# mjiUST/SurfaceNet

Hardware: AMD Instinct MI355X
Metric: voxel-cubes/sec (CVC warp + 3D CNN fwd) at s=32, N_viewpair=2 (higher is better)
Workload: dtype f16x3 (each operand = hi+lo fp16 pair, 3 MFMAs per product, f32 accumulate: fp32-class results; the two correction terms of a product run on one MX-scaled MFMA in the two merge layers (fp6 e2m3 codes) and in the three dilated layers conv4_x (fp8 e4m3 codes); L_inf vs fp64 oracle 3e-5 .. 1.7e-4, asse; 1 GPU; synthetic 2-view 1600x1200, s=32, batch=64 cubes/GPU, N_viewpair=2 (BASELINE.json configs[1]); cubes_per_gpu=64, parallelism=cube-sharded x1

## Files before the change

surfacenet_amd/csrc/conv3d_mfma.h:

```cpp
#pragma once
#include <hip/hip_runtime.h>
#include "mx_format.h"
#include <stdint.h>
#include <type_traits>

constexpr int kRowGap3x3 = 4, kRowGap2D = 4, kRowGapDil2 = 2;
#ifndef SN_TIMING
#define SN_TIMING 0
#endif
#define PW_SB __builtin_amdgcn_sched_barrier(0)

namespace sn {

typedef _Float16 half8 __attribute__((ext_vector_type(8)));
typedef _Float16 half4 __attribute__((ext_vector_type(4)));
typedef float f32x4 __attribute__((ext_vector_type(4)));

constexpr int kMaxSlab = 128;

struct ConvArgs {
    const _Float16 *in;
    _Float16 *out;
    float *out_f32;
    const _Float16 *wpack;
    const float *scale;
    const float *shift;
    const float *w3;
    const void *zero_page;
    const _Float16 *side_w;
    const float *side_scale, *side_shift;
    _Float16 *side_out, *pool_out;
    long long side_lo_off, pool_lo_off;
    int side_cs, side_coff, pool_cs, side_act;
    unsigned *status;
    unsigned status_bit;
    unsigned mx_sat_bits;
    float scale3, shift3;
    long long wsplit_stride;
    long long in_lo_off, out_lo_off;
    long long out_code_off;
    int in_cs, out_cs, out_coff, out_cp;
    int D, DX, tiles_x, tiles_y, tiles_z, total_tiles;
    int act;
    int mx_in_e8, mx_out_e8, mx_side_e8;
    int nslab;
    int c8_last;
    int bridge;
};

enum { EPI_STORE = 0, EPI_FINAL = 1, EPI_POOL2D = 2, EPI_SIDEPOOL = 3 };

template <int V> struct IntC { static constexpr int value = V; };
__device__ __forceinline__ float sn_sigmoid(float x) { return 1.0f / (1.0f + __expf(-x)); }
typedef float f32x2_t __attribute__((ext_vector_type(2)));
__device__ __forceinline__ void sn_track_acc(f32x2_t &c, const f32x4 &a)
// ... 93 lines not shown
__device__ __forceinline__ void pw_mfma_f16(f32x4 &c, const half8 &a, const half8 &b)
{
    asm volatile("v_mfma_f32_16x16x32_f16 %0, %1, %2, %0" : "+a"(c) : "v"(a), "v"(b));
}
template <int OPSEL>
__device__ __forceinline__ void pw_mfma_mx6(f32x4 &c, const mx_v6i &a, const mx_v6i &b, int sa, int sb)
{
    static_assert(OPSEL >= 0 && OPSEL < 4, "scale byte");
#define SN_MX6_ASM(SEL) "v_mfma_scale_f32_16x16x128_f8f6f4 %0, %1, %2, %0, %3, %4 " SEL " cbsz:" SN_STR(SN_MX_FMT) " blgp:" SN_STR(SN_MX_FMT)
    if constexpr (OPSEL == 0) asm volatile(SN_MX6_ASM("op_sel_hi:[0,0,0]") : "+a"(c) : "v"(a), "v"(b), "v"(sa), "v"(sb));
    else if constexpr (OPSEL == 1) asm volatile(SN_MX6_ASM("op_sel:[1,0,0] op_sel_hi:[0,0,0]") : "+a"(c) : "v"(a), "v"(b), "v"(sa), "v"(sb));
    else if constexpr (OPSEL == 2) asm volatile(SN_MX6_ASM("op_sel_hi:[1,0,0]") : "+a"(c) : "v"(a), "v"(b), "v"(sa), "v"(sb));
    else asm volatile(SN_MX6_ASM("op_sel:[1,0,0] op_sel_hi:[1,0,0]") : "+a"(c) : "v"(a), "v"(b), "v"(sa), "v"(sb));
#undef SN_MX6_ASM
}
__device__ __forceinline__ void pw_mfma_mx8(f32x4 &c, const v8i &a, const v8i &b, int sa, int sb)
{
    asm volatile("v_mfma_scale_f32_16x16x128_f8f6f4 %0, %1, %2, %0, %3, %4 op_sel_hi:[0,0,0]" : "+a"(c) : "v"(a), "v"(b), "v"(sa), "v"(sb));
}
constexpr unsigned HB_ALWAYS = 1u << 31, HB_XLO = 1u << 30, HB_XHI = 1u << 29, HB_YLO = 1u << 28, HB_YHI = 1u << 27, HB_ZLO = 1u << 26,
                   HB_ZHI = 1u << 25, HB_OFFMASK = (1u << 25) - 1;

template <int KS, int DIL, int MF, int NF, int EPI, int SPLIT, int CS8, int PCH_, int NW_, int PADV_, int K2D = 0>
struct ConvCfg {
    static constexpr int R = (KS / 2) * DIL;
    static constexpr int RX = K2D ? 0 : R;
    static constexpr int XS = MF / 4;
    static constexpr int NW = NW_;
    static constexpr int NT = NW * 64;
    static constexpr bool F4 = (K2D == 2);
    static constexpr int TX = F4 ? NW * MF : NW * XS, TY = F4 ? 4 : 8, TZ = F4 ? 4 : 8;
    static constexpr int HX = TX + 2 * RX, HY = TY + 2 * R, HZ = TZ + 2 * R;
    static constexpr int HVOX = HX * HY * HZ;
    static constexpr int CS8MAX = CS8;
    static constexpr int SLOTS = CS8 + PADV_;
    static constexpr int VS = SLOTS * 16;
    static constexpr int PCH = PCH_;
    static constexpr int NPL = SPLIT ? 2 : 1;
    static constexpr int NPLM = SPLIT == 1 ? 2 : 1;
    static constexpr int FRAG = 1024 * NPL;
    static constexpr int MFRAG = 1024 * NPLM;
    static_assert(SPLIT < 2 || PCH_ == 2, "f16m8: a weight piece is 2 K-chunks + one MX step");
    static constexpr int MXF = SPLIT == 3 ? 0 : SN_MX_FMT;
    static constexpr int WBUF = PCH * NF * FRAG;
    static constexpr int NTAP = (K2D ? 1 : KS) * KS * KS;
    static constexpr int KOFF_N = NTAP * CS8MAX + 24;
    static constexpr bool PWM = (SPLIT == 3 || (SPLIT == 2 && SN_MX_FMT != 0)) && K2D == 0 && NW_ == 4 && KS == 3 && MF == 8 && PCH_ == 2;
    static constexpr int PW_TABS = 16;
    static constexpr int pw_tab(int kb, int slab, bool last) { return kb * PW_TABS + (last ? 8 : 0) + (slab & 7); }
    static constexpr int pw_xoff(int m) { return (((m >> 2) * HY + (m & 3)) * HZ) * VS; }
    static constexpr int XGAP = DIL == 2 ? kRowGapDil2 : kRowGap3x3;
    static constexpr int xoff_of(int m) { return XGAP == 4 ? pw_xoff(m) : (((m >> 2) * HY + (m & 1) + 4 * ((m >> 1) & 1)) * HZ) * VS; }
    static constexpr bool PTAB = SPLIT < 2 && NW_ == 8 && KS == 3 && PCH_ >= 2 && (K2D == 0 || SPLIT != 0) && !PWM;
    static constexpr int KTAB_N = PWM ? PW_TABS * KOFF_N : (PTAB ? 8 * KOFF_N : KOFF_N);
    static constexpr int NSEG0 = (HVOX * VS + 1023) / 1024;
    static constexpr int NSEG = PWM ? (NSEG0 + NW_ - 1) / NW_ * NW_ : NSEG0;
    static constexpr int XPLANE = NSEG * 1024;
    static constexpr int XBUF = XPLANE * NPL;
#ifndef SN_PW_WB3
#define SN_PW_WB3 0
#endif
    static constexpr bool CST_LDS = (EPI == EPI_STORE) && NF >= 7;
    static constexpr int EPI_CONST = CST_LDS ? NF * 16 * 4 * 2 : 0;
    static constexpr int NWB = (SN_PW_WB3 && PWM && 2 * XBUF + 3 * WBUF + 2 * KTAB_N * 4 + EPI_CONST <= 160 * 1024) ? 3 : 2;
    static constexpr int wb_next(int b) { return NWB == 3 ? (b == 2 ? 0 : b + 1) : (b ^ 1); }
    static constexpr int LDS_BYTES = 2 * XBUF + NWB * WBUF + 2 * KTAB_N * 4 + EPI_CONST;
    static_assert(LDS_BYTES <= 160 * 1024, "LDS budget exceeded");
    static constexpr int WG_PER_CU = (LDS_BYTES <= 80 * 1024 && NW == 4 && MF * NF <= 32) ? 2 : 1;
    static constexpr int MIN_WAVES_PER_SIMD = (NW == 8 || WG_PER_CU == 2) ? 2 : 1;
};

template <int KS, int SPLIT, int NW, int PCH, int NF, int K2D, int MF = 4>
constexpr bool sn_conv_has_bridge()
{
    return (SPLIT == 1 && NW == 8 && KS == 3 && PCH >= 2) ||
           (SPLIT == 2 && K2D == 0 && NW == 8 && KS == 3 && SN_MX_FMT != 0) ||
           ((SPLIT == 3 || (SPLIT == 2 && SN_MX_FMT != 0)) && K2D == 0 && NW == 4 && MF == 8 && KS == 3 && PCH == 2);
}

template <int KS, int DIL, int MF, int NF, int EPI, int SPLIT, int CS8, int PCH_, int NW_, int PADV_, int K2D = 0, int OSPLIT_ = -1>
__global__ void __launch_bounds__(NW_ * 64, (ConvCfg<KS, DIL, MF, NF, EPI, SPLIT, CS8, PCH_, NW_, PADV_, K2D>::MIN_WAVES_PER_SIMD))
conv3d_f16_mfma(ConvArgs a)
{
    constexpr int OSPLIT = OSPLIT_ < 0 ? SPLIT : OSPLIT_;
    using C = ConvCfg<KS, DIL, MF, NF, EPI, SPLIT, CS8, PCH_, NW_, PADV_, K2D>;
    constexpr int NPL = C::NPL;
    __shared__ __attribute__((aligned(16))) char lds[C::LDS_BYTES];
    char *const xbuf = lds;
    char *const wbuf = lds + 2 * C::XBUF;
    int *const kbuf = reinterpret_cast<int *>(lds + 2 * C::XBUF + C::NWB * C::WBUF);
    float *const cst = reinterpret_cast<float *>(lds + 2 * C::XBUF + C::NWB * C::WBUF + 2 * C::KTAB_N * 4);

    const int tid = threadIdx.x, lane = tid & 63, wave = __builtin_amdgcn_readfirstlane(tid >> 6);
    const int v = lane & 15, kq = lane >> 4;
    int mx_sb = a.mx_in_e8;
    if constexpr (SPLIT == 3 || (SPLIT == 2 && SN_MX_FMT != 0)) asm volatile("" : "+v"(mx_sb));
    const int D = a.D, DX = a.DX;
    const size_t VOL = (size_t)DX * D * D;
    const int tstride = gridDim.x;
    auto slab_c8_of = [&](int sl) -> int { return sl + 1 == a.nslab ? a.c8_last : C::CS8MAX; };
    int tile = ((gridDim.x & 7) == 0) ? (int)((blockIdx.x & 7) * (gridDim.x >> 3) + (blockIdx.x >> 3)) : (int)blockIdx.x;
    if (tile >= a.total_tiles) return;

    const char *const wsrc0 = reinterpret_cast<const char *>(a.wpack + (size_t)blockIdx.y * a.wsplit_stride);

    auto tile_origin = [&](int t, int &b, int &x0, int &y0, int &z0) {
        const int tz = t % a.tiles_z; t /= a.tiles_z;
        const int ty = t % a.tiles_y; t /= a.tiles_y;
        const int tx = t % a.tiles_x;
        b = t / a.tiles_x;
        x0 = tx * C::TX; y0 = ty * C::TY; z0 = tz * C::TZ;
// ... 54 lines not shown
            }
            hword[k] = o;
        });
    }
    auto tile_halo_consts = [&](int x0, int y0, int z0, unsigned &keep, int &toff) {
        unsigned inv = K2D ? 0u : HB_ALWAYS;
        if constexpr (K2D == 0) {
            if (x0 == 0) inv |= HB_XLO;
            if (x0 == (a.tiles_x - 1) * C::TX) inv |= HB_XHI;
        }
        if (y0 == 0) inv |= FB_YLO;
        if (y0 == (a.tiles_y - 1) * C::TY) inv |= FB_YHI;
        if (z0 == 0) inv |= FB_ZLO;
        if (z0 == (a.tiles_z - 1) * C::TZ) inv |= FB_ZHI;
        keep = FB_OFFMASK | inv;
        toff = K2D ? ((y0 - C::R) * D + (z0 - C::R)) * 16 : (((x0 - C::RX) * D + (y0 - C::R)) * D + (z0 - C::R)) * 16;
    };
    auto stage_halo_buf = [&](int b, unsigned keep, int toff, int c0, int c8n, int xb, int kb = 0, int ke = 1 << 20) -> int {
        if constexpr (UNI) {
            b = __builtin_amdgcn_readfirstlane(b); keep = __builtin_amdgcn_readfirstlane(keep);
            toff = __builtin_amdgcn_readfirstlane(toff); c0 = __builtin_amdgcn_readfirstlane(c0);
        }
        asm volatile("" : "+s"(b), "+s"(keep), "+s"(toff), "+s"(c0));
        const char *base0;
        int nrec;
        if constexpr (K2D == 0) {
            base0 = reinterpret_cast<const char *>(a.in) + 2 * ((size_t)b * VOL * a.in_cs + (size_t)c0 * VOL * 8);
            nrec = c8n * (int)VOL * 16;
        } else {
            base0 = reinterpret_cast<const char *>(a.in) + 2 * ((size_t)c0 * VOL * 8 + (size_t)b * D * D * 8);
            nrec = (c8n * (int)VOL - b * D * D) * 16;
        }
        if constexpr (UNI) {
            const unsigned long long bq = (unsigned long long)(size_t)base0;
            base0 = (const char *)(size_t)(((unsigned long long)(unsigned)__builtin_amdgcn_readfirstlane((int)(bq >> 32)) << 32) |
                                           (unsigned)__builtin_amdgcn_readfirstlane((int)bq));
            nrec = __builtin_amdgcn_readfirstlane(nrec);
        }
        int issued = 0;
        static_for<0, HT>([&](auto kc) {
            constexpr int k = decltype(kc)::value;
            const int li = k * C::NW + wave;
            if ((k + 1 < HT || C::NSEG * NPL == HT * C::NW || li < C::NSEG * NPL) && k >= kb && k < ke) {
                const char *base = (NPL > 1 && li >= C::NSEG) ? base0 + 2 * a.in_lo_off : base0;
                const __amdgpu_buffer_rsrc_t rs = __builtin_amdgcn_make_buffer_rsrc((void *)base, (short)0, nrec, 0x00020000);
                dma16_buf(rs, (hword[k] & keep) + (unsigned)toff, xbuf + xb * C::XBUF + li * 1024);
                ++issued;
            }
        });
        return issued;
    };
    auto wg_barrier = [&]() { asm volatile("s_barrier" ::: "memory"); };
    constexpr bool BRIDGE_OK = (PPX && SPLIT == 1) || PPM || PWM;
    constexpr int UM = SPLIT >= 2 ? 8 : 4;
    constexpr int BSTEP = (UM - (C::NTAP * C::CS8MAX) % UM) % UM;
    const bool bridge = BRIDGE_OK && a.bridge != 0;
    auto slab_units = [&](int c8n, int slab, int &o, int &b) {
        const int GU = C::NTAP * c8n;
        o = 0; b = 0;
        if (bridge) {
            o = (slab * ((UM - (GU & (UM - 1))) & (UM - 1))) & (UM - 1);
            b = (slab + 1 == a.nslab) ? 0 : ((UM - ((GU - o) & (UM - 1))) & (UM - 1));
        }
        return GU - o + b;
    };
    auto chunks_of = [&](int c8n, int slab) { int o, b; return (slab_units(c8n, slab, o, b) + 3) >> 2; };
    auto wchunks_of = [&](int c8n, int slab) { int o, b; return SPLIT >= 2 ? (((slab_units(c8n, slab, o, b) + 7) >> 3) << 1) : chunks_of(c8n, slab); };
    const int wchunk0 = wchunks_of(slab_c8_of(0), 0);
    auto write_koff_part = [&](int c8n, int kb, int slab, int t0, int nt) {
        int uo, ub;
        const int own = slab_units(c8n, slab, uo, ub) - ub, nchunk = (own + ub + 3) >> 2;
        int *k = kbuf + (PWM ? C::pw_tab(kb, slab, slab + 1 == a.nslab) : (C::PTAB ? kb * 8 + ((slab + 1 == a.nslab) ? 4 : 0) + (slab & 3) : kb)) * C::KOFF_N;
        for (int g = t0; g < (nchunk + 4) * 4; g += nt) {
            int o = 0;
            if (g < own + ub) {
                const int u = g < own ? g + uo : g - own;
                const int far = g < own ? 0 : (1 - 2 * kb) * C::XBUF;
                const int tap = C::CS8MAX == 1 ? u : u / c8n, c8 = C::CS8MAX == 1 ? 0 : u - tap * c8n;
                const int dz = tap % KS, dy = (tap / KS) % KS, dx = tap / (KS * KS);
                o = ((dx * DIL * C::HY + dy * DIL) * C::HZ + dz * DIL) * C::VS + c8 * 16 + far;
            }
            k[g] = o;
        }
    };
    auto write_koff = [&](int c8n, int kb, int slab) { write_koff_part(c8n, kb, slab, tid, C::NT); };
    auto stage_w = [&](size_t off, int nch, int wbi) {
        const int cnt = nch * NF * NPL;
        const char *src = wsrc0 + off;
        char *dst = wbuf + wbi * C::WBUF;
        for (int i = wave; i < cnt; i += C::NW) dma16(src + (size_t)i * 1024 + lane * 16, dst + i * 1024);
    };

    constexpr bool PMAP = (EPI == EPI_SIDEPOOL);
    static_assert(!PMAP || ((MF == 4 || MF == 8) && NW_ == 8 && K2D == 0), "EPI_SIDEPOOL: 8 waves x 4 (8) fragments over an 8x8x8 (16x8x8) tile");
    auto frag_xyz = [&](int m, int &hx, int &hy, int &hz) {
        if constexpr (C::F4) { hx = wave * MF + m; hy = v >> 2; hz = v & 3; }
        else if constexpr (PMAP) { hx = (MF / 2) * (wave & 3) + (m >> 1); hy = 2 * (wave >> 2) + (m & 1) + 4 * (v >> 3); hz = v & 7; }
        else if constexpr (K2D == 0 && KS == 3 && C::XGAP == 4) { hx = wave * C::XS + (m >> 2); hy = (m & 3) + 4 * (v >> 3); hz = v & 7; }
        else if constexpr (K2D == 0 && KS == 3 && C::XGAP == 2) { hx = wave * C::XS + (m >> 2); hy = (m & 1) + 4 * ((m >> 1) & 1) + 2 * (v >> 3); hz = v & 7; }
        else if constexpr (K2D == 1 && kRowGap2D == 4 && C::VS == 32) { hx = wave * C::XS + (m >> 2); hy = (m & 3) + 4 * (v >> 3); hz = v & 7; }
        else { hx = wave * C::XS + (m >> 2); hy = 2 * (m & 3) + (v >> 3); hz = v & 7; }
    };
    int xbase[MF];
#pragma unroll
    for (int m = 0; m < MF; ++m) {
        int hx, hy, hz;
        frag_xyz(m, hx, hy, hz);
        xbase[m] = ((hx * C::HY + hy) * C::HZ + hz) * C::VS;
    }
    const unsigned xbuf_a = lds_addr(xbuf), wbuf_a = lds_addr(wbuf) + lane * 16, kbuf_a = lds_addr(kbuf) + kq * 4;

    if constexpr (C::CST_LDS)
        for (int i = tid; i < NF * 16; i += C::NT) {
            cst[i] = a.scale[blockIdx.y * NF * 16 + i];
            cst[NF * 16 + i] = a.shift[blockIdx.y * NF * 16 + i];
        }
    constexpr int NQ = (NF + 1) / 2;
    half8 sw[EPI == EPI_SIDEPOOL ? NQ : 1][2];
    if constexpr (EPI == EPI_SIDEPOOL) {
#pragma unroll
        for (int q = 0; q < NQ; ++q) {
            sw[q][0] = *reinterpret_cast<const half8 *>(a.side_w + ((size_t)(q * 2 + 0) * 64 + lane) * 8);
            sw[q][1] = *reinterpret_cast<const half8 *>(a.side_w + ((size_t)(q * 2 + 1) * 64 + lane) * 8);
        }
    }
    {
        const int c8n = slab_c8_of(0);
        if constexpr (BUFH) {
            int b, x0, y0, z0, toff;
            unsigned keep;
            tile_origin(tile, b, x0, y0, z0);
            tile_halo_consts(x0, y0, z0, keep, toff);
            stage_halo_buf(K2D ? x0 : b, keep, toff, 0, c8n, 0);
        } else stage_halo(tile, 0, c8n, 0, 0, HT);
        if constexpr (C::PTAB) {
            for (int kb = 0; kb < 2; ++kb)
// ... 1018 lines not shown
```

surfacenet_amd/csrc/sn_api.hip:

```cpp
#include "sn_internal.h"

enum Kind { K_CONV3, K_CONV1, K_DIL3, K_DIL1, K_UP };
struct LayerSpec { const char *name; Kind kind; int cin, cout, act; const char *input; };
static const LayerSpec kSpecs[] = {
    {"conv1_1", K_CONV3, 6, 32, 0, nullptr},       {"conv1_2", K_CONV3, 32, 32, 0, "conv1_1"},    {"conv1_3", K_CONV3, 32, 32, 0, "conv1_2"},
    {"side_op1", K_CONV1, 32, 16, 1, "conv1_3"},
    {"conv2_1", K_CONV3, 32, 80, 0, "conv1_3"},    {"conv2_2", K_CONV3, 80, 80, 0, "conv2_1"},    {"conv2_3", K_CONV3, 80, 80, 0, "conv2_2"},
    {"side_op2", K_CONV1, 80, 16, 1, "conv2_3"},   {"side_op2_deconv", K_UP, 3, 2, 0, nullptr},
    {"conv3_1", K_CONV3, 80, 160, 0, "conv2_3"},   {"conv3_2", K_CONV3, 160, 160, 0, "conv3_1"},  {"conv3_3", K_CONV3, 160, 160, 0, "conv3_2"},
    {"side_op3", K_CONV1, 160, 16, 1, "conv3_3"},  {"side_op3_deconv", K_UP, 5, 4, 0, nullptr},
    {"conv4_1", K_DIL3, 160, 300, 0, "conv3_3"},   {"conv4_2", K_DIL3, 300, 300, 0, "conv4_1"},   {"conv4_3", K_DIL3, 300, 300, 0, "conv4_2"},
    {"side_op4", K_DIL1, 300, 16, 1, "conv4_3"},   {"side_op4_deconv", K_UP, 5, 4, 0, nullptr},
    {"merge_conv_a", K_CONV3, 64, 100, 0, nullptr}, {"merge_conv_b", K_CONV3, 100, 100, 0, "merge_conv_a"}, {"merge_conv3", K_CONV1, 100, 1, 1, "merge_conv_b"},
};
static constexpr int kNumSpecs = sizeof(kSpecs) / sizeof(kSpecs[0]);
static constexpr int kNetParams = 98, kAllParams = 105, kDFeature = 258, kHidden = 100;


static unsigned char fp8_e4m3(float v)
{
    if (v != v) return 0x7f;
    const unsigned char sgn = std::signbit(v) ? 0x80 : 0;
    float a = std::fabs(v);
    if (a >= 448.f) return sgn | 0x7e;
    if (a < std::ldexp(1.0f, -10)) return sgn;
    int e;
    std::frexp(a, &e);
    int E = e - 1;
    if (E < -6) E = -6;
    const float q = std::nearbyint(std::ldexp(a, 3 - E));
    int mant = (int)q, be = E + 7;
    if (E == -6 && mant < 8) be = 0;
    else { if (mant == 16) { mant = 8; be += 1; } mant -= 8; }
    if (be > 15 || (be == 15 && mant > 6)) return sgn | 0x7e;
    return sgn | (unsigned char)(be << 3) | (unsigned char)mant;
}

static unsigned char mx6_encode(float v, int fmt)
{
    const int mb = fmt == 2 ? 3 : 2, bias = fmt == 2 ? 1 : 3, emax = fmt == 2 ? 3 : 7;
    const float vmax = std::ldexp((float)((2 << mb) - 1), emax - bias - mb);
    if (v != v) return 0;
    const unsigned char sgn = std::signbit(v) ? 0x20 : 0;
    float a = std::min(std::fabs(v), vmax);
    int e;
    std::frexp(a, &e);
    int E = (a > 0.f) ? e - 1 : 1 - bias;
    if (E < 1 - bias) E = 1 - bias;
    int mant = (int)std::nearbyint(std::ldexp(a, mb - E));
    int be = E + bias;
    if (mant < (1 << mb)) be = 0;
    else { if (mant == (2 << mb)) { mant = 1 << mb; be += 1; } mant -= 1 << mb; }
    if (be > emax) { be = emax; mant = (1 << mb) - 1; }
    return sgn | (unsigned char)(be << mb) | (unsigned char)mant;
}
static float mx6_max(int fmt) { return fmt == 2 ? 7.5f : 28.f; }

static int pack_conv_host(PackedConv &L, const float *W_in, const float *beta, const float *gamma, const float *mean,
                          const float *inv_std, int nf, int nsplit, int cs8max, int split, const int *in_exp, const int *out_exp,
                          std::vector<_Float16> &h, std::vector<float> &sc, std::vector<float> &sh)
{
    L.nf = nf; L.nsplit = nsplit; L.cs8max = cs8max; L.split = split;
    L.cin_p = round_up(L.cin, 8);
    const int ntap = (L.k2d ? 1 : L.ks) * L.ks * L.ks;
    const int c8_total = L.cin_p / 8;
    const int npl = split == 1 ? 2 : 1;
    L.slab_c8.clear();
    for (int left = c8_total; left > 0; left -= cs8max) L.slab_c8.push_back((unsigned char)std::min(left, cs8max));
    if ((int)L.slab_c8.size() > kMaxSlab) return fail(SN_ERR_ARG, "%s: too many channel slabs", L.name.c_str());
    std::vector<float> Wn((size_t)L.cout * L.cin * ntap);
    std::vector<int> row_exp(L.cout, 0);
    for (int o = 0; o < L.cout; ++o) {
        float mx = 0.f;
        for (int ci = 0; ci < L.cin; ++ci)
            for (int t = 0; t < ntap; ++t) {
                const size_t i = ((size_t)o * L.cin + ci) * ntap + t;
                const float w = in_exp ? std::ldexp(W_in[i], -in_exp[ci]) : W_in[i];
                if (!std::isfinite(w)) return fail(SN_ERR_ARG, "%s: non-finite weight (output channel %d, input channel %d)", L.name.c_str(), o, ci);
                Wn[i] = w;
                mx = std::max(mx, std::fabs(w));
            }
        if (mx > 0.f) row_exp[o] = -std::ilogb(mx);
        if (row_exp[o] != 0)
            for (size_t i = (size_t)o * L.cin * ntap; i < (size_t)(o + 1) * L.cin * ntap; ++i) Wn[i] = std::ldexp(Wn[i], row_exp[o]);
    }
    if (ntap == 1) L.w_norm = Wn;
    const float *W = Wn.data();
    auto wat = [&](int o, int c8abs, int j, int tap) -> float {
        const int ci = c8abs * 8 + j;
        return (o < L.cout && ci < L.cin) ? W[((size_t)o * L.cin + ci) * ntap + tap] : 0.f;
    };
    h.clear();
    {
        const int um = split >= 2 ? 8 : 4;
        bool ok = L.bridge && (split == 1 || (split >= 2 && !L.k2d)) && L.ks == 3 && L.slab_c8.size() >= 2 && (ntap * cs8max) % um != 0;
        for (unsigned char c8n : L.slab_c8) ok = ok && c8n == cs8max;
        L.bridge = ok ? 1 : 0;
    }
    const int nslab = (int)L.slab_c8.size();
    auto slab_units = [&](int si, int c8n, int &o, int &b) {
        const int GU = ntap * c8n, um = split >= 2 ? 8 : 4;
        o = 0; b = 0;
        if (L.bridge) { o = (si * ((um - GU % um) % um)) % um; b = (si + 1 == nslab) ? 0 : (um - (GU - o) % um) % um; }
        return GU - o + b;
    };
    if (split < 2) {
        long long chunks = 0;
        for (int si = 0; si < nslab; ++si) { int o, b; chunks += (slab_units(si, L.slab_c8[si], o, b) + 3) / 4; }
        L.wsplit_stride = chunks * nf * 512 * npl;
        h.assign((size_t)L.wsplit_stride * nsplit, (_Float16)0.f);
        for (int ns = 0; ns < nsplit; ++ns) {
            _Float16 *dst = h.data() + (size_t)ns * L.wsplit_stride;
            int c8_0 = 0;
            for (int si = 0; si < nslab; ++si) {
                const int c8n = L.slab_c8[si];
                int uo, ub;
                const int own = slab_units(si, c8n, uo, ub) - ub, nchunk = (own + ub + 3) / 4;
                for (int ch = 0; ch < nchunk; ++ch)
                    for (int f = 0; f < nf; ++f)
                        for (int lane = 0; lane < 64; ++lane) {
                            const int o = (ns * nf + f) * 16 + (lane & 15);
                            const int g = 4 * ch + (lane >> 4);
                            _Float16 *d8 = dst + (((size_t)ch * nf + f) * npl * 64 + lane) * 8;
                            if (g >= own + ub) continue;
                            const int u = g < own ? g + uo : g - own;
                            const int cb = g < own ? c8_0 : c8_0 + c8n;
                            for (int j = 0; j < 8; ++j) {
                                const float w = wat(o, cb + u % c8n, j, u / c8n);
                                const _Float16 hi = (_Float16)w;
                                d8[j] = hi;
                                if (split == 1) d8[512 + j] = (_Float16)(w - (float)hi);
                            }
                        }
                dst += (size_t)nchunk * nf * 512 * npl;
                c8_0 += c8n;
            }
        }
    } else {
        long long pieces = 0;
        for (int si = 0; si < nslab; ++si) { int o, b; pieces += (slab_units(si, L.slab_c8[si], o, b) + 7) / 8; }
        const size_t piece_halfs = (size_t)nf * 2048;
        L.wsplit_stride = pieces * piece_halfs;
        h.assign((size_t)L.wsplit_stride * nsplit, (_Float16)0.f);
        for (int ns = 0; ns < nsplit; ++ns) {
            _Float16 *dst = h.data() + (size_t)ns * L.wsplit_stride;
            int c8_0 = 0;
            for (int si = 0; si < nslab; ++si) {
                const int c8n = L.slab_c8[si];
                int uo, ub;
                const int own = slab_units(si, c8n, uo, ub) - ub, G = own + ub, npiece = (G + 7) / 8;
                auto wslot = [&](int o, int g, int j) -> float {
                    const int u = g < own ? g + uo : g - own, cb = g < own ? c8_0 : c8_0 + c8n;
                    return wat(o, cb + u % c8n, j, u / c8n);
                };
                for (int p = 0; p < npiece; ++p, dst += piece_halfs) {
                    for (int cc = 0; cc < 2; ++cc)
                        for (int f = 0; f < nf; ++f)
                            for (int lane = 0; lane < 64; ++lane) {
                                const int o = (ns * nf + f) * 16 + (lane & 15);
                                const int g = 8 * p + 4 * cc + (lane >> 4);
                                if (g >= G) continue;
                                _Float16 *d8 = dst + (((size_t)cc * nf + f) * 64 + lane) * 8;
                                for (int j = 0; j < 8; ++j) d8[j] = (_Float16)wslot(o, g, j);
                            }
                    unsigned char *mx = reinterpret_cast<unsigned char *>(dst + (size_t)2 * nf * 512);
                    for (int f = 0; f < nf; ++f)
                        for (int lane = 0; lane < 64; ++lane) {
                            const int o = (ns * nf + f) * 16 + (lane & 15), q = lane >> 4;
                            unsigned char *frag = mx + (size_t)f * 2048;
                            if (split == 2) {
                                float val[32];
                                float amax = 0.f;
                                for (int i = 0; i < 2; ++i) {
                                    const int g = 8 * p + 2 * q + i;
                                    for (int pos = 0; pos < 16; ++pos) {
                                        const int j = (pos & 3) + 4 * (pos >> 3);
                                        const bool lo_part = !(pos & 4);
                                        float t = 0.f;
                                        if (g < G) {
                                            const float w = wslot(o, g, j);
                                            const float hi = (float)(_Float16)w;
                                            t = lo_part ? (w - hi) * kMxLoMul : hi;
                                        }
                                        val[i * 16 + pos] = t;
                                        amax = std::max(amax, std::fabs(t));
                                    }
                                }
                                int E = 0;
                                if (amax > 0.f) {
                                    E = std::ilogb(amax / mx6_max(SN_MX_FMT));
                                    if (std::ldexp(amax, -E) > mx6_max(SN_MX_FMT)) ++E;
                                }
                                E = std::max(-100, std::min(100, E));
                                unsigned w6[6] = {0u, 0u, 0u, 0u, 0u, 0u};
                                for (int el = 0; el < 32; ++el) {
                                    const unsigned code = mx6_encode(std::ldexp(val[el], -E), SN_MX_FMT);
                                    const int bit = 6 * el;
                                    w6[bit >> 5] |= code << (bit & 31);
                                    if ((bit & 31) > 26) w6[(bit >> 5) + 1] |= code >> (32 - (bit & 31));
                                }
                                unsigned *d0 = reinterpret_cast<unsigned *>(frag + lane * 16), *d1 = reinterpret_cast<unsigned *>(frag + 1024 + lane * 16);
                                d0[0] = w6[0]; d0[1] = w6[1]; d0[2] = w6[2]; d0[3] = w6[3];
                                d1[0] = w6[4]; d1[1] = w6[5];
                                (mx + 1024 + lane * 16 + 8)[f] = (unsigned char)std::max(0, std::min(254, 127 + E - kMxLoExp));
                                continue;
// ... 1163 lines not shown
int sn_mark(sn_ctx *c, int slot)
{
    if (!c || slot < 0 || slot >= 8) return fail(SN_ERR_ARG, "sn_mark: slot must be 0..7");
    HIPCHK(hipSetDevice(c->device));
    if (!c->marks[slot]) HIPCHK(hipEventCreateWithFlags(&c->marks[slot], hipEventDisableTiming));
    HIPCHK(hipEventRecord(c->marks[slot], c->stream));
    return SN_OK;
}

int sn_memcpy_d2h_after(sn_ctx *c, int slot, void *dst, const void *src, size_t bytes)
{
    if (!c || !dst || !src) return fail(SN_ERR_ARG, "null argument");
    if (slot < 0 || slot >= 8 || !c->marks[slot]) return fail(SN_ERR_STATE, "sn_memcpy_d2h_after: slot %d was never marked", slot);
    HIPCHK(hipSetDevice(c->device));
    if (!c->copy_stream) HIPCHK(hipStreamCreateWithFlags(&c->copy_stream, hipStreamNonBlocking));
    HIPCHK(hipStreamWaitEvent(c->copy_stream, c->marks[slot], 0));
    HIPCHK(hipMemcpyAsync(dst, src, bytes, hipMemcpyDeviceToHost, c->copy_stream));
    HIPCHK(hipStreamSynchronize(c->copy_stream));
    return SN_OK;
}

#ifdef SN_DEBUG_HOOKS
SN_API int sn_debug_tensor(sn_ctx *c, const char *name, void *host, size_t bytes)
{
    if (!c || !name || !host) return fail(SN_ERR_ARG, "null argument");
    const _Float16 *p = !strcmp(name, "cat") ? c->cat : (!strcmp(name, "ma") ? c->ma : nullptr);
    if (!p) return fail(SN_ERR_ARG, "unknown tensor %s", name);
    HIPCHK(hipSetDevice(c->device));
    HIPCHK(hipStreamSynchronize(c->stream));
    HIPCHK(hipMemcpy(host, p, bytes, hipMemcpyDeviceToHost));
    return SN_OK;
}

SN_API int sn_debug_pack_host(int cin, int cout, int ks, int dil, int k2d, int nf, int nsplit, int cs8max, int split, const float *W, const float *beta,
                              const float *gamma, const float *mean, const float *inv_std, unsigned long long *out)
{
    if (!W || !beta || !gamma || !mean || !inv_std || !out) return fail(SN_ERR_ARG, "null argument");
    PackedConv L;
    L.name = "debug"; L.cin = cin; L.cout = cout; L.ks = ks; L.dil = dil; L.k2d = k2d;
    L.bridge = 1;
    std::vector<_Float16> h;
    std::vector<float> sc, sh;
    const int rc = pack_conv_host(L, W, beta, gamma, mean, inv_std, nf, nsplit, cs8max, split, nullptr, nullptr, h, sc, sh);
    if (rc != SN_OK) return rc;
    unsigned long long sum = 0;
    const unsigned char *b = reinterpret_cast<const unsigned char *>(h.data());
    for (size_t i = 0; i < h.size() * sizeof(_Float16); ++i) sum = sum * 1099511628211ull + b[i];
    out[0] = h.size(); out[1] = sc.size(); out[2] = sh.size(); out[3] = sum;
    return SN_OK;
}

SN_API int sn_debug_plan(int net, int mode, int conv4_fp8, char *rows, int cap)
{
    if (!rows || cap < 1 || net < 0 || net > 1) return fail(SN_ERR_ARG, "sn_debug_plan: bad argument");
    sn_ctx st;
    int rc = sn_set_precision(&st, mode), n = 0;
    if (rc == SN_OK && conv4_fp8 >= 0) rc = sn_set_conv4_fp8(&st, conv4_fp8);
    if (rc != SN_OK) return rc;
    for (const ConvEntry &e : net == 0 ? build_plan(st.split, st.tail_m8, st.c4_m8).conv : simil_plan(st.split)) {
        n += snprintf(rows + n, (size_t)(cap - n), "%s %d %d %d %d %d %d %d %d %d %d %d %d\n", e.name, e.cin, e.cout, e.k.ks, e.k.dil, e.k.k2d,
                      e.k.nf, e.k.nsplit(e.cout), e.k.cs8max, e.k.split, e.k.osplit, e.k.epi, e.bridge);
        if (n >= cap) return fail(SN_ERR_ARG, "sn_debug_plan: the rows do not fit %d bytes", cap);
    }
    return SN_OK;
}

SN_API int sn_debug_mx6_encode(float v, int fmt) { return (fmt == 2 || fmt == 3) ? (int)mx6_encode(v, fmt) : -1; }

SN_API int sn_debug_timing(sn_ctx *c, unsigned long long *out, int n_layers, char *names, int names_cap)
{
    if (!c || !out || !c->d_num) return fail(SN_ERR_ARG, "null argument");
    HIPCHK(hipStreamSynchronize(c->stream));
    n_layers = std::min(n_layers, 32);
    HIPCHK(hipMemcpy(out, c->d_num + 2, sizeof(unsigned long long) * 4 * n_layers, hipMemcpyDeviceToHost));
    HIPCHK(hipMemset(c->d_num + 2, 0, sizeof(unsigned) * 32 * 8));
    std::string all;
    for (auto &nm : c->num_names) all += nm + ",";
    if (names && names_cap > 0) { strncpy(names, all.c_str(), names_cap - 1); names[names_cap - 1] = 0; }
    return SN_OK;
}
SN_API int sn_debug_trace(sn_ctx *c, long long *out)
{
    if (!c || !out || !c->d_num) return fail(SN_ERR_ARG, "null argument");
    HIPCHK(hipStreamSynchronize(c->stream));
    HIPCHK(hipMemcpy(out, c->d_num + 2 + 32 * 8, sizeof(long long) * 2048 * 8 * 2, hipMemcpyDeviceToHost));
    return SN_OK;
}

#endif

int sn_profile_enable(sn_ctx *c, int on)
{
    if (!c) return fail(SN_ERR_ARG, "null context");
    int rc = prof_drain(c);
    c->prof_on = on != 0;
    return rc;
}
int sn_profile_reset(sn_ctx *c)
{
    if (!c) return fail(SN_ERR_ARG, "null context");
    int rc = prof_drain(c);
    for (auto &st : c->prof_stats) { st.ms = 0; st.launches = 0; st.flops = 0; st.bytes = 0; }
    return rc;
}
int sn_profile_count(sn_ctx *c)
{
    if (!c) return fail(SN_ERR_ARG, "null context");
    if (prof_drain(c) != SN_OK) return SN_ERR_HIP;
    return (int)c->prof_stats.size();
}
int sn_profile_get(sn_ctx *c, int idx, char *name, int name_cap, double *ms_total, int64_t *launches, double *flops, double *bytes)
// ... 16 lines not shown
```

surfacenet_amd/csrc/sn_internal.h:

```cpp
#pragma once
#include <hip/hip_runtime.h>
#include <dlfcn.h>

#include <algorithm>
#include <chrono>
#include <cmath>
#include <condition_variable>
#include <memory>
#include <mutex>
#include <thread>
#include <type_traits>
#include <cstdarg>
#include <cstdio>
#include <cstring>
#include <map>
#include <string>
#include <vector>

#include "../../include/surfacenet_hip.h"
#include "conv3d_mfma.h"
#include "cvc_warp.h"
#include "elementwise.h"

using namespace sn;

inline thread_local std::string g_err;

static int fail(int code, const char *fmt, ...)
{
    char buf[1024];
    va_list ap;
    va_start(ap, fmt);
    vsnprintf(buf, sizeof buf, fmt, ap);
    va_end(ap);
    g_err = buf;
    return code;
}

#define HIPCHK(expr)                                                                                       \
    do {                                                                                                   \
        hipError_t e_ = (expr);                                                                            \
        if (e_ != hipSuccess) return fail(SN_ERR_HIP, "%s failed: %s (%s:%d)", #expr, hipGetErrorString(e_), __FILE__, __LINE__); \
    } while (0)


static inline int round_up(int x, int m) { return (x + m - 1) / m * m; }


struct PackedConv {
    std::string name;
    int cin = 0, cout = 0, ks = 1, dil = 1, act = 0;
    int cin_p = 0;
    int nf = 0, nsplit = 1;
    int cs8max = 4, split = 0, k2d = 0;
    int bridge = 0;
    std::vector<unsigned char> slab_c8;
    long long wsplit_stride = 0;
    _Float16 *wpack = nullptr;
    float *scale = nullptr, *shift = nullptr;
    double macs_per_voxel = 0;
    std::vector<float> w_norm;
    _Float16 *side_frag = nullptr;
};

struct sn_ctx;
enum MxExp : unsigned char { MX_ACT, MX_CAT, MX_X0, MX_C4 };

struct Act { _Float16 *p; long long lo; long long code = 0; MxExp e8 = MX_ACT; };

struct SideFuse { const PackedConv *side; Act side_out; int side_cs, side_coff; Act pool_out; int pool_cs; };

struct ConvGeom {
    int ks, dil, k2d, nf, cs8max, split, osplit, epi;
    bool has_bridge;
    int (*launch)(sn_ctx *c, const PackedConv &L, Act in, int in_cs, Act out, int out_cs, int out_coff, int out_cp, float *out_f32, int B, int D, int DX, const SideFuse *sf);
    int nsplit(int cout) const { return ((cout + 15) / 16 + nf - 1) / nf; }
};

struct ConvEntry {
    const char *name; int cin, cout, act;
    ConvGeom k;
    int bridge;
    unsigned char in = 0, out = 0, pool_out = 0;
    const char *pool_tag = nullptr;
    bool up3 = false;
};
struct TensorSpec { _Float16 *sn_ctx::*buf; int level, ch; MxExp e8; int code; };
struct NetPlan {
    int split = -1, tail_m8 = 0, c4_m8 = 0;
    std::vector<ConvEntry> conv;
    std::vector<TensorSpec> tens;
    int (*pool)(sn_ctx *, const char *, Act, Act, int, int, int) = nullptr;
    int (*up3)(sn_ctx *, Act, Act, Act, Act, int, int, int) = nullptr;
};

struct ProfRec { int tag; hipEvent_t e0, e1; double flops, bytes; };
struct ProfStat { std::string name; double ms = 0; int64_t launches = 0; double flops = 0, bytes = 0; };

static inline const char *sn_ab_switch(const char *name)
{
#ifdef SN_DEBUG_HOOKS
    return getenv(name);
#else
    (void)name;
    return nullptr;
#endif
}

constexpr int CC_ERR_INPUT_FLAG = 2;

struct sn_ctx {
    int device = 0, s = 32, max_samples = 0;
    hipStream_t stream = nullptr;
    hipStream_t copy_stream = nullptr;
    hipEvent_t marks[8] = {};
    int V_img = 0, V_cam = 0;
    uint8_t *img_base = nullptr; long long *img_off = nullptr; int *img_h = nullptr, *img_w = nullptr;
    double *cams = nullptr;
    bool have_weights = false, have_relw = false;
    int split = 1;
    int mode = 1;
    int mx_c4_e8 = kMxC4E8;
    int c4_m8 = 1;
    _Float16 *a3c = nullptr;
    int mx_act_e8 = kMxActE8, mx_cat_e8 = kMxCatE8;
    int tail_m8 = 2;
    bool ws_ready = false; int ws_split = -1;
    int last_run_samples = 0;
    NetPlan plan;
// ... 143 lines not shown
                return fail(SN_ERR_ARG, "%s: volume extent %d is not supported by this kernel's halo addressing (extent mod 8 must be 0 or >= %d)", L.name.c_str(), D, C::R);
            const long long plane = (long long)DX * D * D * 16, slack = 4LL * C::HVOX * 16;
            if (K2D == 0 && C::CS8MAX * plane + slack >= (1LL << 25))
                return fail(SN_ERR_ARG, "%s: a %d-group channel slab of a %dx%dx%d volume exceeds the 32 MiB this kernel's halo addressing covers", L.name.c_str(), C::CS8MAX, DX, D, D);
            if (K2D != 0 && SPLIT != 0 && C::CS8MAX * plane + slack >= 0x0FFFFFF0LL - (1 << 16))
                return fail(SN_ERR_ARG, "%s: %d images of %dx%d exceed the 256 MiB this kernel's halo addressing covers per channel slab", L.name.c_str(), DX, D, D);
        }
        a.act = L.act;
        if (EPI == EPI_STORE && KS != 1 && L.act != 0)
            return fail(SN_ERR_STATE, "%s: a sigmoid activation is only built for the 1x1x1 store kernels", L.name.c_str());
        a.mx_in_e8 = mx_e8(c, in.e8); a.mx_out_e8 = mx_e8(c, out.e8); a.mx_side_e8 = mx_e8(c, sf ? sf->side_out.e8 : MX_ACT);
        if (EPI == EPI_SIDEPOOL) {
            if (!sf || !sf->side || !sf->side->side_frag || sf->side->cin != L.cout || sf->side->cout != 16 || L.nsplit != 1 || L.act != 0 || (D & 1))
                return fail(SN_ERR_STATE, "%s: fused side-conv / pool epilogue misconfigured", L.name.c_str());
            a.side_w = sf->side->side_frag; a.side_scale = sf->side->scale; a.side_shift = sf->side->shift; a.side_act = sf->side->act;
            a.side_out = sf->side_out.p; a.side_lo_off = sf->side_out.lo; a.side_cs = sf->side_cs; a.side_coff = sf->side_coff;
            a.pool_out = sf->pool_out.p; a.pool_lo_off = sf->pool_out.lo; a.pool_cs = sf->pool_cs;
        }
        if (c->d_num) {
            auto it = std::find(c->num_names.begin(), c->num_names.end(), L.name);
            size_t bit = it - c->num_names.begin();
            if (it == c->num_names.end() && c->num_names.size() < 31) c->num_names.push_back(L.name);
            a.status = c->d_num;
            constexpr int OS = OSPLIT < 0 ? SPLIT : OSPLIT;
            if (EPI == EPI_STORE && OS >= 2 && L.act == 0) {
                const _Float16 lim = (_Float16)std::min(60000.f, std::ldexp(OS >= 3 ? 255.875f : (SN_MX_FMT == 2 ? 7.5f : 28.f), a.mx_out_e8 - 127));
                unsigned short bits; memcpy(&bits, &lim, 2);
                a.mx_sat_bits = bits;
            }
            a.status_bit = bit < 31 ? (1u << bit) : (1u << 31);
        }
        a.nslab = (int)L.slab_c8.size();
        if (a.nslab < 1) return fail(SN_ERR_STATE, "%s: no channel slabs", L.name.c_str());
        a.bridge = L.bridge;
        if (L.bridge && !geom.has_bridge)
            return fail(SN_ERR_STATE, "%s: packed with bridge chunks, launched on a kernel without them", L.name.c_str());
        if (C::PWM) {
            for (unsigned char c8n : L.slab_c8)
                if (C::NTAP * c8n < 9) return fail(SN_ERR_STATE, "%s: a channel slab of fewer than two weight pieces", L.name.c_str());
        }
        for (int i = 0; i + 1 < a.nslab; ++i)
            if (L.slab_c8[i] != C::CS8MAX) return fail(SN_ERR_STATE, "%s: channel slab %d holds %d groups, the kernel expects %d in all but the last", L.name.c_str(), i, (int)L.slab_c8[i], C::CS8MAX);
        a.c8_last = L.slab_c8.back();
        const double vox = (double)B * DX * D * D;
        const double bytes = vox * 2.0 * (SPLIT ? 2 : 1) * (L.cin + (EPI == EPI_FINAL ? 2 : (EPI == EPI_SIDEPOOL ? 16 + L.cout / 8.0 : L.cout)));
        ProfScope ps(c, L.name, 2.0 * L.macs_per_voxel * vox, bytes);
        const int resident = std::max(1, c->num_cus * C::WG_PER_CU / L.nsplit);
        dim3 grid((unsigned)std::min(a.total_tiles, resident), (unsigned)L.nsplit);
        hipLaunchKernelGGL((conv3d_f16_mfma<KS, DIL, MF, NF, EPI, SPLIT, CS8, PCH, NW, PADV, K2D, OSPLIT>), grid, dim3(NW * 64), 0, c->stream, a);
        HIPCHK(hipGetLastError());
        return SN_OK;
    }
    static constexpr ConvGeom geom = {KS, DIL, K2D != 0, NF, C::CS8MAX, SPLIT, OSPLIT < 0 ? SPLIT : OSPLIT, EPI,
                                      sn::sn_conv_has_bridge<KS, SPLIT, NW, PCH, NF, K2D, MF>(), &launch};
};

struct TmpDev {
    std::vector<void *> p;
    ~TmpDev() { for (void *q : p) (void)hipFree(q); }
    template <typename T> T *get(size_t count) { void *q = nullptr; if (hipMalloc(&q, std::max<size_t>(count, 1) * sizeof(T)) != hipSuccess) return nullptr; p.push_back(q); return static_cast<T *>(q); }
};
```

Before: 7607 cubes/s.

## Reorder conv taps into quad groups for single-channel-group 3x3x3 layers

Adds a fixed tap permutation for 3x3x3 convolutions with one 8-channel group per slab (dilation 1 and 2). Taps are grouped into quads and a triple, and both the host weight packer and the device LDS offset tables follow this order. Padding entries in partial chunks now repeat real offsets instead of pointing at zero. The apparent aim is better LDS access locality or fewer bank conflicts within each MFMA chunk. A debug-plan dump of the tables is also added, and packing and kernel tables must stay consistent.

```diff
diff --git a/surfacenet_amd/csrc/conv3d_mfma.h b/surfacenet_amd/csrc/conv3d_mfma.h
--- a/surfacenet_amd/csrc/conv3d_mfma.h
+++ b/surfacenet_amd/csrc/conv3d_mfma.h
@@ -1,6 +1,7 @@
 #pragma once
 #include <hip/hip_runtime.h>
 #include "mx_format.h"
+#include "tap_order.h"
 #include <stdint.h>
 #include <type_traits>
 
@@ -200,11 +201,15 @@
     static constexpr int XGAP = DIL == 2 ? kRowGapDil2 : kRowGap3x3;
     static constexpr int xoff_of(int m) { return XGAP == 4 ? pw_xoff(m) : (((m >> 2) * HY + (m & 1) + 4 * ((m >> 1) & 1)) * HZ) * VS; }
     static constexpr bool PTAB = SPLIT < 2 && NW_ == 8 && KS == 3 && PCH_ >= 2 && (K2D == 0 || SPLIT != 0) && !PWM;
+    static constexpr int LOOP = PWM ? 3 : ((SPLIT == 2 && K2D == 0 && NW_ == 8 && KS == 3 && SN_MX_FMT != 0) ? 2 : (PTAB ? 1 : 0));
+    static constexpr int ROWMAP = F4 ? 0 : ((EPI == EPI_SIDEPOOL || (K2D == 0 && KS == 3)) ? (EPI == EPI_SIDEPOOL ? 4 : XGAP) : ((K2D == 1 && kRowGap2D == 4 && VS == 32) ? 4 : 1));
     static constexpr int KTAB_N = PWM ? PW_TABS * KOFF_N : (PTAB ? 8 * KOFF_N : KOFF_N);
     static constexpr int NSEG0 = (HVOX * VS + 1023) / 1024;
     static constexpr int NSEG = PWM ? (NSEG0 + NW_ - 1) / NW_ * NW_ : NSEG0;
     static constexpr int XPLANE = NSEG * 1024;
     static constexpr int XBUF = XPLANE * NPL;
+    static constexpr int UM = SPLIT >= 2 ? 8 : 4;
+    static constexpr TapGeom tap_geom() { return TapGeom{KS, DIL, K2D != 0, HY, HZ, VS, CS8MAX, XBUF, UM, NTAP}; }
 #ifndef SN_PW_WB3
 #define SN_PW_WB3 0
 #endif
@@ -365,7 +370,7 @@
     };
     auto wg_barrier = [&]() { asm volatile("s_barrier" ::: "memory"); };
     constexpr bool BRIDGE_OK = (PPX && SPLIT == 1) || PPM || PWM;
-    constexpr int UM = SPLIT >= 2 ? 8 : 4;
+    constexpr int UM = C::UM;
     constexpr int BSTEP = (UM - (C::NTAP * C::CS8MAX) % UM) % UM;
     const bool bridge = BRIDGE_OK && a.bridge != 0;
     auto slab_units = [&](int c8n, int slab, int &o, int &b) {
@@ -381,20 +386,9 @@
     auto wchunks_of = [&](int c8n, int slab) { int o, b; return SPLIT >= 2 ? (((slab_units(c8n, slab, o, b) + 7) >> 3) << 1) : chunks_of(c8n, slab); };
     const int wchunk0 = wchunks_of(slab_c8_of(0), 0);
     auto write_koff_part = [&](int c8n, int kb, int slab, int t0, int nt) {
-        int uo, ub;
-        const int own = slab_units(c8n, slab, uo, ub) - ub, nchunk = (own + ub + 3) >> 2;
+        const int nchunk = chunks_of(c8n, slab);
         int *k = kbuf + (PWM ? C::pw_tab(kb, slab, slab + 1 == a.nslab) : (C::PTAB ? kb * 8 + ((slab + 1 == a.nslab) ? 4 : 0) + (slab & 3) : kb)) * C::KOFF_N;
-        for (int g = t0; g < (nchunk + 4) * 4; g += nt) {
-            int o = 0;
-            if (g < own + ub) {
-                const int u = g < own ? g + uo : g - own;
-                const int far = g < own ? 0 : (1 - 2 * kb) * C::XBUF;
-                const int tap = C::CS8MAX == 1 ? u : u / c8n, c8 = C::CS8MAX == 1 ? 0 : u - tap * c8n;
-                const int dz = tap % KS, dy = (tap / KS) % KS, dx = tap / (KS * KS);
-                o = ((dx * DIL * C::HY + dy * DIL) * C::HZ + dz * DIL) * C::VS + c8 * 16 + far;
-            }
-            k[g] = o;
-        }
+        for (int g = t0; g < (nchunk + 4) * 4; g += nt) k[g] = g < nchunk * 4 ? sn_koff_entry(C::tap_geom(), c8n, kb, slab, a.nslab, bridge, g) : 0;
     };
     auto write_koff = [&](int c8n, int kb, int slab) { write_koff_part(c8n, kb, slab, tid, C::NT); };
     auto stage_w = [&](size_t off, int nch, int wbi) {
diff --git a/surfacenet_amd/csrc/sn_api.hip b/surfacenet_amd/csrc/sn_api.hip
--- a/surfacenet_amd/csrc/sn_api.hip
+++ b/surfacenet_amd/csrc/sn_api.hip
@@ -55,6 +55,14 @@
     return sgn | (unsigned char)(be << mb) | (unsigned char)mant;
 }
 static float mx6_max(int fmt) { return fmt == 2 ? 7.5f : 28.f; }
+
+static bool bridge_granted(int wanted, int ks, int k2d, int split, int cs8max, const std::vector<unsigned char> &slab_c8)
+{
+    const int um = split >= 2 ? 8 : 4, ntap = (k2d ? 1 : ks) * ks * ks;
+    bool ok = wanted && (split == 1 || (split >= 2 && !k2d)) && ks == 3 && slab_c8.size() >= 2 && (ntap * cs8max) % um != 0;
+    for (unsigned char c8n : slab_c8) ok = ok && c8n == cs8max;
+    return ok;
+}
 
 static int pack_conv_host(PackedConv &L, const float *W_in, const float *beta, const float *gamma, const float *mean,
                           const float *inv_std, int nf, int nsplit, int cs8max, int split, const int *in_exp, const int *out_exp,
@@ -91,18 +99,18 @@
         return (o < L.cout && ci < L.cin) ? W[((size_t)o * L.cin + ci) * ntap + tap] : 0.f;
     };
     h.clear();
-    {
-        const int um = split >= 2 ? 8 : 4;
-        bool ok = L.bridge && (split == 1 || (split >= 2 && !L.k2d)) && L.ks == 3 && L.slab_c8.size() >= 2 && (ntap * cs8max) % um != 0;
-        for (unsigned char c8n : L.slab_c8) ok = ok && c8n == cs8max;
-        L.bridge = ok ? 1 : 0;
-    }
+    L.bridge = bridge_granted(L.bridge, L.ks, L.k2d, split, cs8max, L.slab_c8) ? 1 : 0;
     const int nslab = (int)L.slab_c8.size();
     auto slab_units = [&](int si, int c8n, int &o, int &b) {
         const int GU = ntap * c8n, um = split >= 2 ? 8 : 4;
         o = 0; b = 0;
         if (L.bridge) { o = (si * ((um - GU % um) % um)) % um; b = (si + 1 == nslab) ? 0 : (um - (GU - o) % um) % um; }
         return GU - o + b;
+    };
+    auto unit_at = [&](int si, int c8n, int g, int own, int uo) {
+        int no = 0, nb = 0;
+        if (g >= own) slab_units(si + 1, c8n, no, nb);
+        return g < own ? sn::sn_tap_unit(L.ks, L.dil, L.k2d, c8n, uo & 3, g + uo) : sn::sn_tap_unit(L.ks, L.dil, L.k2d, c8n, no & 3, g - own);
     };
     if (split < 2) {
         long long chunks = 0;
@@ -123,7 +131,7 @@
                             const int g = 4 * ch + (lane >> 4);
                             _Float16 *d8 = dst + (((size_t)ch * nf + f) * npl * 64 + lane) * 8;
                             if (g >= own + ub) continue;
-                            const int u = g < own ? g + uo : g - own;
+                            const int u = unit_at(si, c8n, g, own, uo);
                             const int cb = g < own ? c8_0 : c8_0 + c8n;
                             for (int j = 0; j < 8; ++j) {
                                 const float w = wat(o, cb + u % c8n, j, u / c8n);
@@ -150,7 +158,7 @@
                 int uo, ub;
                 const int own = slab_units(si, c8n, uo, ub) - ub, G = own + ub, npiece = (G + 7) / 8;
                 auto wslot = [&](int o, int g, int j) -> float {
-                    const int u = g < own ? g + uo : g - own, cb = g < own ? c8_0 : c8_0 + c8n;
+                    const int u = unit_at(si, c8n, g, own, uo), cb = g < own ? c8_0 : c8_0 + c8n;
                     return wat(o, cb + u % c8n, j, u / c8n);
                 };
                 for (int p = 0; p < npiece; ++p, dst += piece_halfs) {
@@ -1420,11 +1428,43 @@
 
 SN_API int sn_debug_plan(int net, int mode, int conv4_fp8, char *rows, int cap)
 {
+    const int layer = net >= 256 ? (net >> 8) - 1 : -1;
+    if (layer >= 0) net &= 255;
     if (!rows || cap < 1 || net < 0 || net > 1) return fail(SN_ERR_ARG, "sn_debug_plan: bad argument");
     sn_ctx st;
     int rc = sn_set_precision(&st, mode), n = 0;
     if (rc == SN_OK && conv4_fp8 >= 0) rc = sn_set_conv4_fp8(&st, conv4_fp8);
     if (rc != SN_OK) return rc;
+    if (layer >= 0) {
+        const std::vector<ConvEntry> plan = net == 0 ? build_plan(st.split, st.tail_m8, st.c4_m8).conv : simil_plan(st.split);
+        if (layer >= (int)plan.size()) return fail(SN_ERR_ARG, "sn_debug_plan: the plan has %d layers", (int)plan.size());
+        const ConvEntry &e = plan[layer];
+        const sn::TapGeom &t = e.k.tg;
+        std::vector<unsigned char> slab_c8;
+        for (int left = round_up(e.cin, 8) / 8; left > 0; left -= t.cs8max) slab_c8.push_back((unsigned char)std::min(left, t.cs8max));
+        const int nslab = (int)slab_c8.size();
+        const bool bridge = bridge_granted(e.bridge, t.ks, t.k2d, e.k.split, t.cs8max, slab_c8);
+        auto put = [&](const char *fmt, ...) {
+            va_list ap;
+            va_start(ap, fmt);
+            if (n < cap) n += vsnprintf(rows + n, (size_t)(cap - n), fmt, ap);
+            va_end(ap);
+        };
+        put("geom %d %d %d %d %d %d %d %d %d %d %d %d %d %d %d %d\n", t.ks, t.dil, t.k2d, t.hy, t.hz, t.vs, t.cs8max, t.xbuf, t.um, t.ntap, e.k.split, e.k.loop, e.k.rowmap,
+            nslab, (int)slab_c8.back(), bridge ? 1 : 0);
+        for (int kb = 0; kb < 2; ++kb)
+            for (int sl = 0; sl < nslab; ++sl) {
+                const int key = e.k.loop == 3 ? 8 : (e.k.loop == 1 ? 4 : 0);
+                const int rep = (key == 0 || sl < key || sl + 1 == nslab) ? sl : sl % key;
+                int uo, ub;
+                const int total = sn::sn_slab_units(t, slab_c8[rep], rep, nslab, bridge, uo, ub), cnt = (total + t.um - 1) / t.um * t.um;
+                put("tab %d %d %d %d %d %d %d", kb, sl, rep, total - ub, uo, ub, cnt);
+                for (int g = 0; g < cnt; ++g) put(" %d", sn::sn_koff_entry(t, slab_c8[rep], kb, rep, nslab, bridge, g));
+                put("\n");
+            }
+        if (n >= cap) return fail(SN_ERR_ARG, "sn_debug_plan: the tables do not fit %d bytes", cap);
+        return SN_OK;
+    }
     for (const ConvEntry &e : net == 0 ? build_plan(st.split, st.tail_m8, st.c4_m8).conv : simil_plan(st.split)) {
         n += snprintf(rows + n, (size_t)(cap - n), "%s %d %d %d %d %d %d %d %d %d %d %d %d\n", e.name, e.cin, e.cout, e.k.ks, e.k.dil, e.k.k2d,
                       e.k.nf, e.k.nsplit(e.cout), e.k.cs8max, e.k.split, e.k.osplit, e.k.epi, e.bridge);
diff --git a/surfacenet_amd/csrc/sn_internal.h b/surfacenet_amd/csrc/sn_internal.h
--- a/surfacenet_amd/csrc/sn_internal.h
+++ b/surfacenet_amd/csrc/sn_internal.h
@@ -75,6 +75,8 @@
     bool has_bridge;
     int (*launch)(sn_ctx *c, const PackedConv &L, Act in, int in_cs, Act out, int out_cs, int out_coff, int out_cp, float *out_f32, int B, int D, int DX, const SideFuse *sf);
     int nsplit(int cout) const { return ((cout + 15) / 16 + nf - 1) / nf; }
+    sn::TapGeom tg;
+    int loop, rowmap;
 };
 
 struct ConvEntry {
@@ -324,7 +326,7 @@
         return SN_OK;
     }
     static constexpr ConvGeom geom = {KS, DIL, K2D != 0, NF, C::CS8MAX, SPLIT, OSPLIT < 0 ? SPLIT : OSPLIT, EPI,
-                                      sn::sn_conv_has_bridge<KS, SPLIT, NW, PCH, NF, K2D, MF>(), &launch};
+                                      sn::sn_conv_has_bridge<KS, SPLIT, NW, PCH, NF, K2D, MF>(), &launch, C::tap_geom(), C::LOOP, C::ROWMAP};
 };
 
 struct TmpDev {
diff --git a/surfacenet_amd/csrc/tap_order.h b/surfacenet_amd/csrc/tap_order.h
--- /dev/null
+++ b/surfacenet_amd/csrc/tap_order.h
@@ -0,0 +1,69 @@
+#pragma once
+
+namespace sn {
+
+constexpr unsigned long long sn_tap_pack12(int t0, int t1, int t2, int t3, int t4, int t5, int t6, int t7, int t8, int t9, int t10, int t11)
+{
+    const int t[12] = {t0, t1, t2, t3, t4, t5, t6, t7, t8, t9, t10, t11};
+    unsigned long long w = 0;
+    for (int i = 0; i < 12; ++i) w |= (unsigned long long)t[i] << (5 * i);
+    return w;
+}
+constexpr unsigned long long kTapQuadsD1a = sn_tap_pack12(16, 15, 19, 18, 10, 7, 11, 8, 4, 3, 17, 20);
+constexpr unsigned long long kTapQuadsD1b = sn_tap_pack12(25, 26, 24, 5, 22, 23, 9, 6, 1, 0, 2, 21);
+constexpr int kTapTripleD1 = 12;
+constexpr unsigned long long kTapQuadsD2a = sn_tap_pack12(7, 25, 16, 1, 6, 8, 0, 2, 9, 15, 18, 24);
+constexpr unsigned long long kTapQuadsD2b = sn_tap_pack12(10, 11, 19, 20, 22, 23, 13, 14, 12, 21, 26, 17);
+constexpr int kTapTripleD2 = 3;
+
+constexpr int sn_tap_order_class(int ks, int dil, int k2d, int c8n) { return (ks == 3 && !k2d && c8n == 1 && (dil == 1 || dil == 2)) ? dil : 0; }
+
+constexpr int sn_tap_unit(int ks, int dil, int k2d, int c8n, int lead, int pos)
+{
+    const int cls = sn_tap_order_class(ks, dil, k2d, c8n);
+    if (cls == 0) return pos;
+    const int j = pos - lead;
+    if (j >= 0 && j < 24) {
+        const unsigned long long w = j < 12 ? (cls == 1 ? kTapQuadsD1a : kTapQuadsD2a) : (cls == 1 ? kTapQuadsD1b : kTapQuadsD2b);
+        return (int)((w >> (5 * (j < 12 ? j : j - 12))) & 31);
+    }
+    const unsigned front = lead == 1 ? 2u : (lead == 2 ? 4u : 18u), back = lead == 0 ? 36u : (lead == 1 ? 4u : 2u);
+    return (cls == 1 ? kTapTripleD1 : kTapTripleD2) + (int)(((j < 0 ? front >> (2 * pos) : back >> (2 * (j - 24)))) & 3u);
+}
+
+struct TapGeom {
+    int ks, dil, k2d, hy, hz, vs, cs8max, xbuf, um, ntap;
+};
+
+constexpr int sn_slab_units(const TapGeom t, int c8n, int slab, int nslab, bool bridge, int &o, int &b)
+{
+    const int GU = t.ntap * c8n, UM = t.um;
+    o = 0; b = 0;
+    if (bridge) {
+        o = (slab * ((UM - (GU & (UM - 1))) & (UM - 1))) & (UM - 1);
+        b = (slab + 1 == nslab) ? 0 : ((UM - ((GU - o) & (UM - 1))) & (UM - 1));
+    }
+    return GU - o + b;
+}
+
+constexpr int sn_koff_entry(const TapGeom t, int c8n, int kb, int slab, int nslab, bool bridge, int g)
+{
+    int uo = 0, ub = 0;
+    const int total = sn_slab_units(t, c8n, slab, nslab, bridge, uo, ub), own = total - ub;
+    if (g >= total) {
+        const int q0 = g & ~3, nreal = total - q0;
+        if (nreal <= 0) return 0;
+        g = nreal == 1 ? q0 : (nreal == 2 ? q0 + (g & 1) : q0 + 2);
+    }
+    const bool mine = g < own;
+    const int pos = mine ? g + uo : g - own;
+    int no = 0, nb = 0;
+    if (!mine) sn_slab_units(t, c8n, slab + 1, nslab, bridge, no, nb);
+    const int u = sn_tap_unit(t.ks, t.dil, t.k2d, c8n, (mine ? uo : no) & 3, pos);
+    const int far = mine ? 0 : (1 - 2 * kb) * t.xbuf;
+    const int tap = t.cs8max == 1 ? u : u / c8n, c8 = t.cs8max == 1 ? 0 : u - tap * c8n;
+    const int dz = tap % t.ks, dy = (tap / t.ks) % t.ks, dx = tap / (t.ks * t.ks);
+    return ((dx * t.dil * t.hy + dy * t.dil) * t.hz + dz * t.dil) * t.vs + c8 * 16 + far;
+}
+
+}
```

Measured after the change: 7596 cubes/s. Within noise of the previous version (-0.1%).
